# noce2/FluidFramework

Measured on AMD Instinct MI355X. Metric: sequenced merge-tree ops applied/sec (node) at 100k docs; bit-exact text+props, higher is better.
Workload: dtype int32; 1 GPU; c3: 100000 docs/GPU x 10000 sequenced ops, 8 writers, refSeq lag <= 64, insert 0.5 / remove 0.3 / annotate 0.2; docs_total=100000, docs_per_gpu=100000, ops_per_doc=10000, parallelism=doc-shard x1

## Files before the change

fluidframework_amd/__init__.py:

```python
import ctypes

import numpy as np

from . import _native
from .wire import CHECKSUM_DTYPE, OP_DTYPE, Batch, Interner

__all__ = ["MergeTreeBatch", "DeviceBatch", "Batch", "Interner", "DeltaLogOverflow"]


class DeltaLogOverflow(RuntimeError):

    def __init__(self, msg, records):
        super().__init__(msg)
        self.records = records


class PinnedArray:

    def __init__(self, lib, n, dtype):
        dt = np.dtype(dtype)
        nbytes = max(int(n), 1) * dt.itemsize
        self.lib = lib
        self.p = lib.mt_host_alloc(nbytes)
        if not self.p:
# ... 354 lines not shown
        off = np.zeros(self.n_docs + 1, dtype=np.int64)
        self._check(self.lib.mt_generated_seeds_docs(self.h, ctypes.byref(c), doc_base, _native.ptr(ids),
                                                     _native.ptr(off), None), "mt_generated_seeds")
        seed = np.zeros(max(int(off[-1]), 1), dtype=np.uint16)
        self._check(self.lib.mt_generated_seeds_docs(self.h, ctypes.byref(c), doc_base, _native.ptr(ids),
                                                     _native.ptr(off), _native.ptr(seed)), "mt_generated_seeds")
        return off, seed

    def sync(self):
        self._check(self.lib.mt_sync(self.h), "mt_sync")

    def last_hbm_docs(self):
        out = np.zeros(8, dtype=np.uint32)
        self._check(self.lib.mt_last_hbm_docs(self.h, _native.ptr(out)), "mt_last_hbm_docs")
        return dict(total=int(out[0]), spilled=int(out[1]), segments=int(out[2]), blocks=int(out[3]), heap=int(out[4]),
                    text=int(out[5]), props=int(out[6]), at_load=int(out[7]))

    def last_paged_peaks(self):
        out = np.zeros(5, dtype=np.uint32)
        self._check(self.lib.mt_last_paged_peaks(self.h, _native.ptr(out)), "mt_last_paged_peaks")
        return dict(pages=int(out[0]), unsettled=int(out[1]), heap=int(out[2]), segments=int(out[3]),
                    tight_handovers=int(out[4]))

    def last_grown(self):
        out = np.zeros(6, dtype=np.uint32)
        self._check(self.lib.mt_last_grown(self.h, _native.ptr(out)), "mt_last_grown")
        return dict(zip(["grown", "rounds", "in_big_region", "pages", "unsettled", "heap"], (int(x) for x in out)))

    def last_kernel_ms(self):
        return float(self.lib.mt_last_kernel_ms(self.h))

    def set_stream_priority(self, priority):
        self._check(self.lib.mt_set_stream_priority(self.h, int(priority)), "mt_set_stream_priority")

    def last_load_ms(self):
        return float(self.lib.mt_last_load_ms(self.h))

    def status(self):
        out = np.zeros(self.n_docs, dtype=np.int32)
        self._check(self.lib.mt_get_status(self.h, _native.ptr(out)), "mt_get_status")
        return out

    def get_length(self, doc):
        out = ctypes.c_uint32()
        self._check(self.lib.mt_get_length(self.h, doc, ctypes.byref(out)), "mt_get_length")
        return out.value
# ... 291 lines not shown
```

fluidframework_amd/_native.py:

```python
import ctypes
import os

import numpy as np

from .wire import CHECKSUM_DTYPE, OP_DTYPE

HERE = os.path.dirname(os.path.abspath(__file__))
MT_E_INVALID, MT_E_HIP, MT_E_NOMEM, MT_E_NODEVICE, MT_E_OVERFLOW, MT_E_STALE_VIEW = -1, -2, -3, -4, -5, -6
LIB_PATH = os.environ.get("MT_LIB_PATH") or os.path.join(HERE, "libmtreplay.so")


class MtOptions(ctypes.Structure):
    _fields_ = [("device", ctypes.c_int32), ("seg_capacity", ctypes.c_int32),
                ("block_capacity", ctypes.c_int32), ("heap_capacity", ctypes.c_int32),
                ("text_capacity", ctypes.c_int32), ("props_capacity", ctypes.c_int32),
                ("delta_log_capacity", ctypes.c_int32), ("lds_seg_capacity", ctypes.c_int32),
                ("page_capacity", ctypes.c_int32), ("page_heap_capacity", ctypes.c_int32),
                ("unsettled_capacity", ctypes.c_int32), ("uid_capacity", ctypes.c_int32),
                ("lds_page_capacity", ctypes.c_int32), ("lds_unsettled_capacity", ctypes.c_int32),
                ("lds_page_heap_capacity", ctypes.c_int32), ("lds_narrow_overlap", ctypes.c_int32),
                ("delta_log_mode", ctypes.c_int32), ("live_client", ctypes.c_int32),
                ("live_group_capacity", ctypes.c_int32), ("paged_slices", ctypes.c_int32),
                ("segment_ordinals", ctypes.c_int32), ("overlap_arena_capacity", ctypes.c_int32)]

# ... 28 lines not shown
    ("mt_num_docs", _U32, [_P]),
    ("mt_load_initial_text", _I, [_P, _P, _P]),
    ("mt_start_collaboration", _I, [_P, _P, _P]),
    ("mt_reset", _I, [_P]),
    ("mt_apply_ops", _I, [_P, _P, _P, _U64, _P, _U64, _P, _U64]),
    ("mt_load_snapshots", _I, [_P, _P, _P, _P, _U64, _P, _U64, _P, _U64, _P, _P]),
    ("mt_extract_snapshots", _I, [_P, _P, _P, _P, _P, _P, _P]),
    ("mt_snapshots_upload", _P, [_P, _P, _P, _P, _U64, _P, _U64, _P, _U64, _P, _P]),
    ("mt_snapshots_upload_range", _P, [_P, _U32, _U32, _P, _P, _P, _U64, _P, _U64, _P, _U64, _P, _P]),
    ("mt_snapshots_load_async", _I, [_P, _P]),
    ("mt_snapshots_free", None, [_P]),
    ("mt_batch_upload", _P, [_P, _P, _P, _U64, _P, _U64, _P, _U64]),
    ("mt_batch_apply_async", _I, [_P, _P]),
    ("mt_batch_num_ops", _U64, [_P]),
    ("mt_batch_free", None, [_P]),
    ("mt_host_alloc", ctypes.c_void_p, [ctypes.c_uint64]),
    ("mt_host_free", None, [ctypes.c_void_p]),
    ("mt_sync", _I, [_P]),
    ("mt_last_kernel_ms", ctypes.c_float, [_P]),
    ("mt_set_stream_priority", ctypes.c_int, [_P, ctypes.c_int]),
    ("mt_last_load_ms", ctypes.c_float, [_P]),
    ("mt_last_hbm_docs", _I, [_P, _P]),
    ("mt_last_paged_peaks", _I, [_P, _P]),
    ("mt_last_grown", _I, [_P, _P]),
    ("mt_generate", _P, [_P, _P, _U32, _P]),
    ("mt_generate_docs", _P, [_P, _P, _U32, _P, _P, _P]),
    ("mt_generated_seeds_docs", _I, [_P, _P, _U32, _P, _P, _P]),
    ("mt_generated_seeds", _I, [_P, _P, _U32, _P, _P]),
    ("mt_batch_sizes", _I, [_P, _P, _P, _P]),
    ("mt_batch_download", _I, [_P, _P, _P, _P, _P]),
    ("mt_get_status", _I, [_P, _P]),
    ("mt_get_length", _I, [_P, _U32, _P]),
    ("mt_get_text", _I, [_P, _U32, _P, _U32, _P]),
    ("mt_get_texts", _I, [_P, _U32, _P, _P, _P, ctypes.c_uint16, _P, _P, _U64]),
    ("mt_get_texts_device", _I, [_P, _U32, _P, _P, _P, ctypes.c_uint16, _P, _P, _U64]),
    ("mt_last_text_ms", _I, [_P, _P]),
    ("mt_get_prop_runs", _I, [_P, _U32, _P, _U32, _P, _P, _U32, _P]),
    ("mt_get_segments", _I, [_P, _U32, _P, _U32, _P, _P, _U32, _P]),
    ("mt_get_segment_props", _I, [_P, _U32, _U32, _P, _U32, _P]),
    ("mt_get_all_segment_props", _I, [_P, _U32, _P, ctypes.c_uint64, _P]),
    ("mt_get_overlap_arena", _I, [_P, _U32, _P]),
    ("mt_get_delta_log", _I, [_P, _U32, _P, _U32, _P]),
    ("mt_delta_log_reset", _I, [_P]),
    ("mt_debug_raw", _I, [_P, _U32, _P, _U32, _P, _P]),
    ("mt_debug_prof", _I, [_P, _P, _I]),
    ("mt_maintenance_counts", _I, [_P, _P]),
# ... 41 lines not shown
```

fluidframework_amd/csrc/mt_device.h:

```cpp
#pragma once
#include <hip/hip_runtime.h>
#include <stdint.h>

#include "../../include/mt_types.h"

#define MT_WAVE 64
#define MT_LV 8
#define MT_MAXN 8
#define MT_HALF 4
#define MT_GRAN 256
#define MT_ZAMBONI 2
#define MT_KMAX 8
#define MT_PREC (1 + 2 * MT_KMAX)
#define MT_RSEQ_NONE ((int32_t)0x80000000)
#define MT_MARKER_BIT 0x80000000u
#define MT_SCOUR_UNDEF ((int8_t)-1)
#define MT_DOC_RETRY 100

typedef unsigned long long u64;
typedef int v4i __attribute__((ext_vector_type(4)));
typedef unsigned v4u __attribute__((ext_vector_type(4)));
typedef int v2i __attribute__((ext_vector_type(2)));

struct DocHdr {
    int32_t n_seg, depth, heap_n, cur_seq;
    int32_t min_seq, text_top, text_half, props_top;
    int32_t props_half, next_uid, status, dlog_n;
    int32_t n_blk[MT_LV];
    u64 delta_hash;
    int32_t n_ops, pad0;
    int32_t pad[8];
};
static_assert(sizeof(DocHdr) == 128, "DocHdr size");
// ... 273 lines not shown
```

fluidframework_amd/csrc/mt_engine.h:

```cpp
#pragma once
#include <type_traits>

#include "mt_device.h"

#define LDS_AS __attribute__((address_space(3)))
#define GLB_AS __attribute__((address_space(1)))

template <bool kLogT> struct TierLdsT {
    static constexpr bool kLds = true;
    static constexpr bool kLog = kLogT;
    static constexpr bool kPaged = false;
    static constexpr bool kLive = false;
    static constexpr int kOvlBits = 32;
    static constexpr bool kMayGrow = false;
    static constexpr bool kOvf = false;
    typedef uint32_t O_v;
    typedef LDS_AS v4i *A_t;
    typedef LDS_AS uint32_t *O_t;
    typedef LDS_AS v4u *B_t;
    typedef LDS_AS v2i *H_t;
};
template <bool kLogT> struct TierGlbT {
    static constexpr bool kLds = false;
    static constexpr bool kLog = kLogT;
// ... 1562 lines not shown
            sa = d.A[s + k];
            so = d.O[s + k];
            sb = d.Bv[s + k];
            if constexpr (T::kLive) sp = pq_get(d, s + k);
            if (ordon(d)) soc = d.os[s + k];
        }
        const int dst = s + __popcll(m_keep & ((1ull << k) - 1ull));
        wsync<T>();
        if (surv) {
            d.A[dst] = sa;
            d.O[dst] = so;
            d.Bv[dst] = sb;
            if constexpr (T::kLive) pq_put(d, dst, sp);
            if (ordon(d)) d.os[dst] = soc;
        }
        wsync<T>();
        if (ordon(d)) gsync();
        seg_move_left(d, e, cntb - keep);
        d.n -= cntb - keep;
    }
    return keep;
}

TD int scour_range(DocT<T> &d, int s, int b0, int nbk) {
    int tot = 0;
    for (int q = 0; q < nbk; q++) tot += cntr(d, 0, b0 + q);
    const int k = lane();
    bool serial = tot > MT_WAVE;
    const bool in = k < tot;
    v4i a = d.A[in ? s + k : s];
    v4u b = d.Bv[in ? s + k : s];
    int start = 0;
    {
        int st = 0;
        for (int q = 0; q < nbk; q++) {
            if (k >= st) start = st;
            st += cntr(d, 0, b0 + q);
        }
    }
    const bool removed = a.z != MT_RSEQ_NONE;
    const bool marker = (b.z & MT_MARKER_BIT) != 0;
    bool pend = false;
    if constexpr (T::kLive) pend = in && pq_any(pq_get(d, in ? s + k : s));
    const bool cand = in && !pend && !removed && a.y <= d.min_seq;
    if (!serial) {
        const bool need_nl = cand && !marker && a.x > 0 && !(b.w & SEGF_NL_KNOWN);
        if (ballot(need_nl)) {
            P2_T0(9)
            gsync_rd();
            if (need_nl) {
                const uint16_t ch = text_base(d, d.text_half)[b.x + a.x - 1];
                b.w = (b.w & ~SEGF_NL) | SEGF_NL_KNOWN | (ch == '\n' ? SEGF_NL : 0u);
                d.Bv[s + k].w = b.w;
            }
            wsync<T>();
            P2_T1(9)
        }
    }
    const u64 m_cand = ballot(cand);
    const u64 m_mark = ballot(in && marker);
    const u64 m_nl = ballot(in && (b.w & SEGF_NL) != 0);
    const uint32_t pprops = (uint32_t)__shfl_up((int)b.y, 1, MT_WAVE);
    const bool pc = k > 0 && ((m_cand >> (k - 1)) & 1ull);
    const bool pm = k > 0 && ((m_mark >> (k - 1)) & 1ull);
    const bool pn = k > 0 && ((m_nl >> (k - 1)) & 1ull);
#ifdef MT_NO_Q4
    const u64 m_nm = 0;
#else
    const u64 m_nm = ballot(in && (b.w & SEGF_NOMATCH) != 0);
#endif
    const bool nm = ((m_nm >> k) & 1ull) || (k > 0 && ((m_nm >> (k - 1)) & 1ull));
    bool join = cand && pc && k != start && !marker && !pm && !pn && a.x > 0;
    if (join && (nm || pprops != b.y)) join = match_props(d, pprops, b.y, nm);
    const u64 m_join = ballot(join);
    if (!serial && ballot(join && a.x > MT_GRAN)) serial = true;
    if (serial) {
        int pos = s, kept_all = 0;
        for (int q = 0; q < nbk; q++) {
            const int old = cntr(d, 0, b0 + q);
            const int kept = scour_block(d, pos, pos + old);
            if (d.status) return kept_all;
            wsync<T>();
            if (lane() == 0) lvl(d, 0)[b0 + q] = (uint8_t)kept;
            wsync<T>();
            pos += kept;
            kept_all += kept;
        }
        return kept_all;
    }
    const bool unlink = in && !pend && removed && a.z <= d.min_seq;
    const bool surv = in && !unlink && !join;
    if (T::kLog) {
        d.m_unlink += __popcll(ballot(unlink));
        d.m_append += __popcll(m_join);
    }
    const u64 m_surv = ballot(surv);
    scour_events(d, a, b, ballot(unlink), m_join, m_surv, s, tot, start);
    const u64 above = (k < 63) ? (m_join >> (k + 1)) : 0ull;
    const u64 m_grp = ballot(surv && (above & 1ull));
    P2_T0(10)
    if (m_grp) {
        mark_dirty(d, s);
        const int L = wave_scan_incl(in ? a.x : 0);
        const int gend = k + __ffsll((long long)~above) - 1;
        const int Lend = __shfl(L, gend < MT_WAVE ? gend : MT_WAVE - 1, MT_WAVE);
        const int glen = Lend - L + (in ? a.x : 0);
        int totc = 0;
        for (u64 g = m_grp; g; g &= g - 1) {
            const int gl = bcast(glen, first_lane(g));
            totc += gl + text_slack(gl);
        }
        if (!text_ensure(d, totc)) return tot;
        gsync_rd();
        for (u64 g = m_grp; g; g &= g - 1) {
            const int kk = first_lane(g);
            const int gk = bcast(glen, kk);
            const int ge = bcast(gend, kk);
            const v4u bk = uni4(d.Bv[s + kk]);
            const int ak = uni(d.A[s + kk].x);
            const uint32_t kslack = bk.w >> SEGF_SLACK_SHIFT;
            const bool mem = k > kk && k <= ge;
            const v4u bm = d.Bv[mem ? s + k : s];
            const int Lm = L - (in ? a.x : 0);
            const int Lk = bcast(L, kk) - ak;
            const int rel = Lm - Lk;
            const bool contig_lane = !mem || (int)bm.x == (int)bk.x + rel;
            const bool contig = !ballot(!contig_lane);
            const int add = gk - ak;
            const uint32_t lastw = (uint32_t)bcast((int)bm.w, ge);
            const uint32_t nonl = (bk.w & SEGF_NONL) && !ballot(mem && !(bm.w & SEGF_NONL)) ? SEGF_NONL : 0u;
            uint32_t newoff = bk.x, newslack = lastw >> SEGF_SLACK_SHIFT;
            if (!contig) {
                int dst;
                bool move_keeper = false;
                if ((uint32_t)add <= kslack) {
                    dst = (int)bk.x + ak;
                    newslack = kslack - (uint32_t)add;
                } else if ((int)bk.x + ak == d.text_top) {
                    dst = d.text_top;
                    newslack = (uint32_t)text_slack(gk);
// ... 1053 lines not shown
```

fluidframework_amd/csrc/mt_kernels.h:

```cpp
#pragma once
#include "../../include/mt_replay.h"
#include "mt_paged.h"

__device__ static void init_doc_hdr(const DevState &st, int doc, int len) {
    DocHdr h;
    memset(&h, 0, sizeof(h));
    h.depth = 1;
    h.n_blk[0] = 1;
    h.text_top = len;
    h.props_top = 1;
    h.next_uid = 2;
    h.delta_hash = MT_FNV_OFF;
    h.status = len > st.T ? MT_DOC_CAPACITY : 0;
    const size_t S = st.S;
    if (len > 0) {
        h.n_seg = 1;
        st.segA[doc * S] = v4i{len, 0, MT_RSEQ_NONE, pack_cli(-1, 0)};
        st.segO[doc * S] = 0ull;
        st.segB[doc * S] = v4u{0u, 0u, 1u, 0u};
        if (st.segP) {
            u64 *w = (u64 *)(st.segP + doc * S);
            w[0] = w[1] = w[2] = w[3] = 0ull;
        }
    }
// ... 387 lines not shown
    gen_end(g, used_out, doc);
    if (T::kLds && d.status == MT_DOC_RETRY) {
        if (lane() == 0) st.retry[doc] = 1;
        return;
    }
    if (lane() == 0) {
        if (d.status) fail_out[doc] = d.status;
        if (!T::kLds) st.retry[doc] = 0;
    }
    store_doc(d, st, doc);
}

template <class T>
__device__ __forceinline__ void pg_peaks(const DevState &st, PagedDoc<T> &pd, int pk_ut, int pk_heap) {
    const int np = nbr(pd.up, 1);
    int ns = 0;
    for (int q = lane(); q < np; q += MT_WAVE) ns += pm_nseg(pd, pd.up.dir[q]);
    ns = wave_sum(ns);
    if (lane() == 0) {
        atomicMax(st.stats + 8, (uint32_t)np);
        atomicMax(st.stats + 9, (uint32_t)pk_ut);
        atomicMax(st.stats + 10, (uint32_t)pk_heap);
        atomicMax(st.stats + 11, (uint32_t)ns);
    }
}
#ifndef MT_PAGED_WAVES
#define MT_PAGED_WAVES 3
#endif
#ifndef MT_HM_WAVES
#define MT_HM_WAVES 2
#endif
#ifndef MT_FULL_WAVES
#define MT_FULL_WAVES 2
#endif
#ifndef MT_PACKED_WAVES
#define MT_PACKED_WAVES 2
#endif
template <class T> constexpr int paged_waves() {
    return T::kHM ? MT_HM_WAVES
                  : (T::kMayGrow ? MT_FULL_WAVES : (T::kPacked ? MT_PACKED_WAVES : MT_PAGED_WAVES));
}
#if MT_PAGED_WAVES > 0
#define MT_PAGED_WPE __attribute__((amdgpu_waves_per_eu(paged_waves<T>())))
#else
#define MT_PAGED_WPE
#endif
// ... 249 lines not shown
```

fluidframework_amd/csrc/mt_paged.h:

```cpp
#pragma once
#include "mt_engine.h"

#ifdef MT_PROF
#define PG_T0(k) const unsigned long long _pt##k = __builtin_amdgcn_s_memtime();
#define PG_T1(k)                                                         \
    if (lane() == 0) {                                                   \
        pd.w.prof[k] += __builtin_amdgcn_s_memtime() - _pt##k;           \
        pd.w.prof[64 + k] += 1ull;                                       \
    }
#define PG_CNT(k)                                                        \
    if (lane() == 0) pd.w.prof[64 + k] += 1ull;
#else
#define PG_T0(k)
#define PG_T1(k)
#define PG_CNT(k)
#endif

template <class T> struct PagedDoc {
    DocT<T> w;
    DocT<T> up;
    LDS_AS PageMeta *meta;
    GLB_AS PageMeta *gmeta;
    LDS_AS int *pvl;
    LDS_AS int *cob;
// ... 43 lines not shown
    int grow;
    int packed;
};

#define PW_B 16
#define MT_PK_MASKS 256

struct PagedLayout {
    uint32_t offWA, offWB, offWO, offWcnt, offWflg, offWends, offWscr, offWnb;
    uint32_t offUcnt, offUnb, offDir, offMeta, offCob, offHeap, offUpage, offUA, offUO, offGen, offProf,
        total;
};
static __host__ __device__ inline PagedLayout paged_layout(int PP, int PH, int UT, int gen_words, int ob,
                                                           bool packed = false, bool hm = false) {
    PagedLayout L;
    uint32_t o = 0;
    L.offWA = o; o += 16u * MT_PG_SLOTS;
    L.offWB = o; o += 16u * MT_PG_SLOTS;
    L.offWO = o; o += (uint32_t)ob * MT_PG_SLOTS;
    L.offUA = o; o += (packed ? 12u : 16u) * UT;
    o = (o + 7u) & ~7u;
    L.offUO = o; o += packed ? 8u * MT_PK_MASKS + MT_PK_MASKS / 8 : ((((uint32_t)ob * UT) + 7u) & ~7u);
    L.offHeap = o; o += 8u * (PH + 1);
    L.offMeta = o; o += hm ? 0u : (uint32_t)sizeof(PageMeta) * PP;
    L.offUpage = o; o += packed ? 0u : (2u * UT + 3u) & ~3u;
    L.offCob = o; o += hm ? 8u * (uint32_t)((PP + 63) / 64) + 4u * 64 : 4u * PP;
    L.offWscr = o; o += 64u * 4;
    L.offWnb = o; o += MT_LV * 4;
    L.offUnb = o; o += MT_LV * 4;
    L.offGen = o; o += 4u * gen_words;
    L.offDir = o; o += 2u * PP;
    L.offWends = o; o += 2u * PW_B;
    L.offWcnt = o; o += (uint32_t)MT_LV * PW_B;
    L.offWflg = o; o += PW_B;
    L.offUcnt = o; o += (uint32_t)(pcnt_bytes(PP) - PP);
#ifdef MT_PROF
    o = (o + 7u) & ~7u;
    L.offProf = o; o += 128u * 8;
#else
    L.offProf = 0;
#endif
    L.total = (o + 15u) & ~15u;
    return L;
}

TD PagedDoc<T> &pdoc(DocT<T> &w) { return *reinterpret_cast<PagedDoc<T> *>(&w); }
template <class T> __device__ __forceinline__ PagedCaps eff_caps(PagedCaps pc) {
// ... 1125 lines not shown
    for (int j = 0; j < nch; j++) {
        const int pg = uni(up.dir[c0 + j]);
        if (lane() == 0) pm_set_ns(pd, pg, 0, 0);
        wsync<T>();
    }
    blk_replace(up, 1, c0, nch, k, base, extra);
    if (up.status) {
        pg_fail_cap(w, 7);
        return;
    }
    for (int m = 0; m < k; m++)
        if (lane() == 0) up.dir[c0 + m] = (uint16_t)newp[m];
    if (lane() == 0) lvl(up, 2)[P] = (uint8_t)k;
    wsync<T>();
    pg_cob_rebuild(pd);
    int top_l = 2, top_b = P;
    if (k < MT_HALF && 3 < up.depth) pack_counts(up, 2, P, top_l, top_b);
    if (up.status) {
        if (w.status == 0) w.cap_cause = up.cap_cause;
        fail(w, MT_DOC_INTERNAL);
        return;
    }
    if (ordon(w)) ord_canon(up, top_l, top_b);
}

TD void pg_zamboni_impl(PagedDoc<T> &pd);
TD void pg_zamboni(PagedDoc<T> &pd) {
    PG_T0(12)
    pg_zamboni_impl(pd);
    PG_T1(12)
}
TD void pg_zamboni_impl(PagedDoc<T> &pd) {
    DocT<T> &w = pd.w;
    pd.vvalid = 0;
    for (int it = 0; it < MT_ZAMBONI && w.status == 0; it++) {
        if (w.heap_n == 0) break;
        const v2i top = heap_top(w);
        if (top.x > w.min_seq) break;
        const uint32_t uid = (uint32_t)top.y;
        if (uid >= (uint32_t)pd.UM) {
            FAIL_INTERNAL(w);
            return;
        }
#ifdef MT_ZPF
        const int gpg = uid == (uint32_t)pd.zuid ? pd.zpv : (int)pd.gumap[uid];
        pd.zuid = 0;
// ... 18 lines not shown
                    PG_CNT(19)
                    continue;
                }
                v4i a = v4i{0, 0, 0, 0};
                u64 o = 0;
                v4u b = v4u{0, 0, 0, 0};
                uint32_t bc = 0, f2 = 0;
                int ob = 0;
                pg_win_fetch(pd, pg, a, o, b);
                pg_win_fetch_blocks(pd, pg, bc, f2, ob);
                if ((((uint32_t)bcast((int)f2, 0)) >> 24) == 0) {
                    PG_CNT(19)
                    continue;
                }
                PG_CNT(18)
                pg_win_flush(pd);
                if (w.status) return;
                pg_win_place(pd, pg, a, o, b, bc, f2, ob);
            } else {
                if (pg == pd.cur || pg >= pd.PP || uni(pm_nseg(pd, pg)) == 0) {
                    PG_CNT(19)
                    continue;
                }
                PG_CNT(18)
                pg_win_switch(pd, pg);
                if (w.status) return;
            }
            i = find_uid(w, uid);
            if (i < 0) {
                PG_CNT(19)
                continue;
            }
        }
        PG_T1(4)
        int bstart;
        const int b = blk_find(w, 0, i, true, bstart);
        if (b < 0) {
            FAIL_INTERNAL(w);
            return;
        }
        const int f = flgr(w, b);
        const int old = cntr(w, 0, b);
        if (f == 0) {
            PG_CNT(20)
            continue;
        }
// ... 175 lines not shown
        const int ns = uni(pm_nseg(pd, pg));
        if (i < ns) {
            GLB_AS v4u *b = pd.gB + (size_t)pg * MT_PG_SLOTS + i;
            const uint32_t nid = (uint32_t)(uni((int)first[pg]) + i);
            v4u bv = *b;
            bv.z = nid | (bv.z & MT_MARKER_BIT);
            *b = bv;
            if (nid < (uint32_t)pd.UM) pd.gumap[nid] = (uint16_t)pg;
        }
    }
    w.next_uid = carry;
    if (w.next_uid + 8 > pd.UM && !soft) pg_fail_cap(w, 9);
    gsync();
    wsync<T>();
}

TD bool pg_room(PagedDoc<T> &pd, const mt_op_rec &op) {
    const bool range = op.kind == MT_OP_REMOVE || op.kind == MT_OP_ANNOTATE;
    const int span = range ? min(max(op.pos2 - op.pos1, 0), 1 << 20) : 0;
    const int ut_b = op.kind == MT_OP_INSERT ? 3 : (range ? 2 + span : (op.kind == MT_OP_LOAD_REMOVED ? 1 : 0));
    const int hp_b = op.kind == MT_OP_INSERT ? 1 : (range ? 1 + span : 0);
    if (T::kOvlBits < 64 && op.kind == MT_OP_REMOVE && oslot_short(pd.w, op_cli(op))) return false;
    if (T::kPacked && op.seq - pd.sbase > 65000) return false;
    if (pd.ut_n + pd.wgrow + ut_b > pd.UT) return false;
    if constexpr (T::kPacked) {
        const int need = pd.wgrow + ut_b;
        if (tab_mfree(pd) < need) {
            tab_mgc(pd);
            if (tab_mfree(pd) < need) return false;
        }
    }
    if (pd.w.heap_n + hp_b > pd.PH) return false;
    if (nbr(pd.up, 1) + 8 > pd.PP) return false;
    for (int l = 2; l < pd.up.depth; l++)
        if (nbr(pd.up, l) + 4 > bcap(pd.up, l)) return false;
    pd.opbound = ut_b;
    pd.wgrow += ut_b;
    return true;
}
TD void pg_apply_op_impl(PagedDoc<T> &pd, const OpIn &in, const GLB_AS uint16_t *tin, const GLB_AS uint32_t *pin);
TD void pg_apply_op(PagedDoc<T> &pd, const OpIn &in, const GLB_AS uint16_t *tin, const GLB_AS uint32_t *pin) {
    PG_T0(15)
    pg_apply_op_impl(pd, in, tin, pin);
    PG_T1(15)
}
TD void pg_load_removed(PagedDoc<T> &pd, const mt_op_rec &op) {
    DocT<T> &w = pd.w;
// ... 549 lines not shown
    pd.upage = (LDS_AS uint16_t *)(smem + L.offUpage);
    pd.uA = (LDS_AS v4i *)(smem + L.offUA);
    pd.uO = (LDS_AS typename T::O_v *)(smem + L.offUO);
    if constexpr (T::kPacked) {
        pd.uL = (LDS_AS uint32_t *)(smem + L.offUA);
        pd.uS = pd.uL + pc.UT;
        pd.uP = pd.uS + pc.UT;
        pd.sbase = h.cur_seq - 32000;
        pd.uM = (LDS_AS u64 *)(smem + L.offUO);
        pd.mbm = (LDS_AS uint32_t *)(smem + L.offUO + 8u * MT_PK_MASKS);
        if (lane() < MT_PK_MASKS / 32) pd.mbm[lane()] = lane() == 0 ? 1u : 0u;
        if (lane() == 0) pd.uM[0] = 0;
    }
    pd.cur = -1;
    pd.cur_pos = -1;
    pd.dirty = 0;
    pd.tdirty = 0;
    pd.vvalid = 0;
    pd.wgrow = 0;
    pd.opbound = 0;
    pd.zuid = 0;
    pd.zpv = 0;
    pd.press = 0;
    pd.ovf_top = MT_OVF_HDR;
    pd.ovf_last = 0;
    pd.ovf_maxn = 0;
    pd.ovf_half = 0;
    pd.ovf_made = 0;
    pd.ovf_peak = 0;
    if constexpr (T::kOvf) {
        if (pd.govf) {
            const GLB_AS uint32_t *hw = (const GLB_AS uint32_t *)pd.govf;
            pd.ovf_top = max((int)hw[0], MT_OVF_HDR);
            pd.ovf_last = (int)hw[1];
            pd.ovf_maxn = (int)hw[2];
            pd.ovf_made = hw[4];
            pd.ovf_peak = (int)hw[5];
            pd.ovf_half = ((int)hw[3] & 1) && pd.ovf_top > mt_ovf_mid(pd.OA) ? 1 : 0;
        }
    }
}

TD void pg_mark_free(PagedDoc<T> &pd) {
    const int np = nbr(pd.up, 1);
    pd.vvalid = 0;
    for (int base = 0; base < pd.PP; base += MT_WAVE)
// ... 300 lines not shown
```

fluidframework_amd/csrc/mt_replay.hip:

```cpp
#include <hip/hip_runtime.h>

#include <algorithm>
#include <cstdlib>
#include <cstdio>
#include <cstring>
#include <string>
#include <vector>

#include "../../include/mt_replay.h"
#include "mt_kernels.h"
#include "mt_variants.h"
#ifdef MT_SINGLE_TU
#define MT_VARIANT_DEF(n, k) const void *mtk_##n() { return (const void *)k; }
MT_VARIANTS(MT_VARIANT_DEF)
#endif

__global__ void __launch_bounds__(MT_WAVE) k_init(DevState st, const int64_t *seed_off,
                                                  const uint16_t *seed) {
    const int doc = blockIdx.x;
    if (doc >= st.n_docs) return;
    oslot_reset(st, doc);
    if (st.bslot && lane() == 0) st.bslot[doc] = -1;
    const int64_t s0 = seed_off ? seed_off[doc] : 0, s1 = seed_off ? seed_off[doc + 1] : 0;
    const int len = (int)(s1 - s0);
// ... 942 lines not shown
            h->pg_resident = per_cu * cus;
        }
    }
    const size_t N = n_docs;
    bool ok = true;
    auto alloc = [&](void **p, size_t bytes) {
        if (!ok) return;
        if (hipMalloc(p, bytes ? bytes : 16) != hipSuccess) ok = false;
    };
    alloc((void **)&st.hdr, N * sizeof(DocHdr));
    alloc((void **)&st.segA, N * st.S * sizeof(int4));
    alloc((void **)&st.segO, N * st.S * sizeof(u64));
    alloc((void **)&st.segB, N * st.S * sizeof(uint4));
    alloc((void **)&st.cnt, N * MT_LV * st.B);
    alloc((void **)&st.flg, N * st.B);
    alloc((void **)&st.heap, N * (size_t)(st.H + 1) * sizeof(int2));
    alloc((void **)&st.oslot, N * (size_t)(2 * MT_OSLOTS) * sizeof(int32_t));
    alloc((void **)&st.text, N * 2 * (size_t)st.T * sizeof(uint16_t));
    alloc((void **)&st.props, N * 2 * (size_t)st.P * MT_PREC * sizeof(uint32_t));
    if (st.DL) alloc((void **)&st.dlog, N * (size_t)st.DL * sizeof(int32_t));
    alloc((void **)&h->d_sums, N * sizeof(mt_checksum));
    alloc((void **)&st.retry, N * sizeof(int32_t));
    alloc((void **)&st.resume, N * sizeof(int64_t));
    alloc((void **)&st.stats, 16 * sizeof(uint32_t));
#ifdef MT_PROF
    alloc((void **)&st.prof, 128 * sizeof(unsigned long long));
    if (ok) ok = hipMemset(st.prof, 0, 128 * sizeof(unsigned long long)) == hipSuccess;
#endif
    if (h->ordinals) {
        alloc((void **)&st.ordS, N * (size_t)st.S * sizeof(uint16_t));
        alloc((void **)&st.ordB, N * (size_t)MT_LV * st.B * sizeof(uint16_t));
    }
    if (h->live) {
        alloc((void **)&st.live, N * 4 * sizeof(int32_t));
        st.LG = std::min(std::max(o.live_group_capacity > 0 ? o.live_group_capacity : 1024, 16), 65535);
        alloc((void **)&st.grp, N * (size_t)(st.LG + 1) * MT_GRP_WORDS * sizeof(int32_t));
        alloc((void **)&st.segP, N * (size_t)st.S * sizeof(PendQ));
    }
    if (st.PP > 0) {
        const size_t slots = N * (size_t)st.PP * MT_PG_SLOTS;
        alloc((void **)&st.pgA, slots * sizeof(int4));
        alloc((void **)&st.pgO, slots * sizeof(u64));
        alloc((void **)&st.pgB, slots * sizeof(uint4));
        alloc((void **)&st.pgMeta, N * st.PP * sizeof(PageMeta));
        alloc((void **)&st.pgDir, N * st.PP * sizeof(uint16_t));
        alloc((void **)&st.pgCnt, N * MT_LV * (size_t)st.PP);
        alloc((void **)&st.pgHeap, N * (size_t)(st.PH + 1) * sizeof(int2));
// ... 233 lines not shown
        launch_replay_paged(MTK(P_LOG), g, blk, lb, h->stream, h->st, b->ops, b->off, b->text,
                           b->props, res, pc, sl);
    else if (pc.narrow)
        launch_replay_paged(MTK(P_NARROW), g, blk, lb, h->stream, h->st, b->ops, b->off,
                           b->text, b->props, res, pc, sl);
    else if (hm)
        launch_replay_paged(MTK(P_HM), g, blk, lb, h->stream, h->st, b->ops, b->off, b->text,
                           b->props, res, pc, sl);
    else
        launch_replay_paged(MTK(P_FULL), g, blk, lb, h->stream, h->st, b->ops, b->off, b->text,
                           b->props, res, pc, sl);
    HIPCHK(h, hipGetLastError());
    return 0;
}

int mt_batch_apply_async(mt_handle *h, const mt_batch *b) {
    if (!h || !b || b->n_docs != h->n_docs) return MT_E_INVALID;
    if (h->pending) {
        const int rc = mt_settle(h);
        if (rc) return rc;
    }
    h->st.order = b->order;
    HIPCHK(h, hipSetDevice(h->device));
    HIPCHK(h, hipMemsetAsync(h->st.stats, 0, 16 * sizeof(uint32_t), h->stream));
    HIPCHK(h, hipEventRecord(h->ev0, h->stream));
    if (h->lds.S > 0) {
        if (h->live && h->st.DL)
            launch_replay(MTK(R_LIVELDS_LOG), dim3(h->n_docs), dim3(MT_WAVE),
                               tier_lds_bytes(true, h->lds, 0), h->stream, h->st, b->ops, b->off, b->text, b->props,
                               h->lds);
        else if (h->live)
            launch_replay(MTK(R_LIVELDS), dim3(h->n_docs), dim3(MT_WAVE),
                               tier_lds_bytes(true, h->lds, 0), h->stream, h->st, b->ops, b->off, b->text, b->props,
                               h->lds);
        else if (h->st.DL)
            launch_replay(MTK(R_LDS_LOG), dim3(h->n_docs), dim3(MT_WAVE), tier_lds_bytes(true, h->lds, 0),
                               h->stream, h->st, b->ops, b->off, b->text, b->props, h->lds);
        else if (h->wpg == 2)
            launch_replay(MTK(R_LDS2), dim3((h->n_docs + 1) / 2), dim3(2 * MT_WAVE),
                               2 * tier_lds_bytes(true, h->lds, 0), h->stream, h->st, b->ops, b->off, b->text, b->props,
                               h->lds);
        else
            launch_replay(MTK(R_LDS), dim3(h->n_docs), dim3(MT_WAVE), tier_lds_bytes(true, h->lds, 0),
                               h->stream, h->st, b->ops, b->off, b->text, b->props, h->lds);
        HIPCHK(h, hipGetLastError());
    } else {
        HIPCHK(h, hipMemsetD32Async((hipDeviceptr_t)h->st.retry, 1, h->n_docs, h->stream));
// ... 564 lines not shown
    HIPCHK(h, hipMemcpy(out, h->st.stats, 8 * sizeof(uint32_t), hipMemcpyDeviceToHost));
    return 0;
}

int mt_last_grown(mt_handle *h, uint32_t *out) {
    if (!h || !out) return MT_E_INVALID;
    SETTLE(h);
    uint32_t in_big = 0;
    for (int32_t x : h->bslot_h) in_big += x >= 0;
    out[0] = h->grown_last;
    out[1] = h->grow_rounds_last;
    out[2] = in_big;
    out[3] = (uint32_t)h->big_caps.PP;
    out[4] = (uint32_t)h->big_caps.UT;
    out[5] = (uint32_t)h->big_caps.PH;
    return 0;
}

int mt_last_paged_peaks(mt_handle *h, uint32_t *out) {
    if (!h || !out) return MT_E_INVALID;
    HIPCHK(h, hipSetDevice(h->device));
    SETTLE(h);
    HIPCHK(h, hipMemcpy(out, h->st.stats + 8, 5 * sizeof(uint32_t), hipMemcpyDeviceToHost));
    return 0;
}

int mt_apply_ops(mt_handle *h, const int64_t *doc_op_off, const mt_op_rec *ops, uint64_t n_ops,
                 const uint16_t *text, uint64_t text_len, const uint32_t *props,
                 uint64_t props_len) {
    if (!h) return MT_E_INVALID;
    h->err.clear();
    mt_batch *b = mt_batch_upload(h, doc_op_off, ops, n_ops, text, text_len, props, props_len);
    if (!b) return h->err.rfind("mt_batch_upload: device", 0) == 0 ? MT_E_NOMEM : MT_E_INVALID;
    int rc = mt_batch_apply_async(h, b);
    if (rc == 0) rc = mt_sync(h);
    mt_batch_free(b);
    return rc;
}

struct mt_snapshots {
    int device = 0;
    uint32_t doc_lo = 0, n_docs = 0;
    int64_t *off = nullptr;
    int32_t *nh = nullptr, *min_seq = nullptr, *cur_seq = nullptr;
    mt_seg_rec *segs = nullptr;
    uint16_t *text = nullptr;
// ... 341 lines not shown
    b->n_ops = off[N];
    b->text_len = off[N] * cfg->text_max + N;
    b->props_len = off[N] * (1 + 2 * (int64_t)cfg->max_keys_per_op) + N;
    int32_t *d_fail = nullptr, *d_trace = nullptr;
    int64_t *d_used = nullptr;
    if (view_len_trace && hipMalloc(&d_trace, std::max<int64_t>(b->n_ops, 1) * 16) != hipSuccess) {
        delete b;
        return nullptr;
    }
    bool ok = hipMalloc(&b->off, (N + 1) * sizeof(int64_t)) == hipSuccess &&
              hipMalloc(&b->ops, std::max<int64_t>(b->n_ops, 1) * sizeof(mt_op_rec)) == hipSuccess &&
              hipMalloc(&b->text, b->text_len * 2) == hipSuccess &&
              hipMalloc(&b->props, b->props_len * 4) == hipSuccess &&
              hipMalloc(&d_fail, N * 4) == hipSuccess && hipMalloc(&d_used, N * 16) == hipSuccess;
    if (ok) {
        ok = hipMemcpy(b->off, off.data(), (N + 1) * 8, hipMemcpyHostToDevice) == hipSuccess &&
             hipMemset(d_fail, 0, N * 4) == hipSuccess && set_order(b, off.data());
        h->st.gen_off = ops_per_doc ? b->off : nullptr;
    }
    int32_t *d_ids = nullptr;
    if (ok && doc_ids)
        ok = hipMalloc(&d_ids, N * 4) == hipSuccess && hipMemcpy(d_ids, doc_ids, N * 4, hipMemcpyHostToDevice) == hipSuccess;
    h->st.gen_ids = d_ids;
    if (ok) ok = hipMemsetAsync(h->st.stats, 0, 16 * sizeof(uint32_t), h->stream) == hipSuccess;
    if (ok) {
        const int gw = 2 * (cfg->writers + 1);
        if (h->lds.S > 0) {
            launch_generate(MTK(G_LDS), dim3(h->n_docs), dim3(MT_WAVE), tier_lds_bytes(true, h->lds, gw),
                               h->stream, h->st, *cfg, doc_index_base, b->ops, b->text, b->props, tstride,
                               pstride, d_fail, d_trace, d_used, h->lds);
            ok = hipGetLastError() == hipSuccess;
        } else {
            ok = hipMemsetD32Async((hipDeviceptr_t)h->st.retry, 1, h->n_docs, h->stream) == hipSuccess;
        }
        if (ok && h->st.PP > 0) {
            const PagedCaps *tiers[2] = {h->pg_tight.PP ? &h->pg_tight : nullptr, &h->pg_full};
            for (const PagedCaps *pc : tiers) {
                if (!pc || !ok) continue;
                const size_t lb = paged_layout(pc->PP, pc->PH, pc->UT, gw, pc->narrow ? 4 : 8).total;
                if (pc->narrow)
                    launch_generate_paged(MTK(GP_NARROW), dim3(h->n_docs), dim3(MT_WAVE), lb,
                                       h->stream, h->st, *cfg, doc_index_base, b->ops, b->text, b->props, tstride,
                                       pstride, d_fail, d_trace, d_used, *pc);
                else
                    launch_generate_paged(MTK(GP_FULL), dim3(h->n_docs), dim3(MT_WAVE), lb,
                                       h->stream, h->st, *cfg, doc_index_base, b->ops, b->text, b->props, tstride,
                                       pstride, d_fail, d_trace, d_used, *pc);
// ... 976 lines not shown
```

include/mt_replay.h:

```cpp
#ifndef MT_REPLAY_H
#define MT_REPLAY_H
#include <stddef.h>
#include <stdint.h>

#include "mt_types.h"

#ifdef __cplusplus
extern "C" {
#endif

#define MT_E_INVALID (-1)
#define MT_E_HIP (-2)
#define MT_E_NOMEM (-3)
#define MT_E_NODEVICE (-4)
#define MT_E_OVERFLOW (-5)
#define MT_E_STALE_VIEW (-6)

typedef struct mt_handle mt_handle;
typedef struct mt_batch mt_batch;

typedef struct mt_options {
    int32_t device;
    int32_t seg_capacity;
    int32_t block_capacity;
// ... 50 lines not shown
                                        const int32_t *n_header, const mt_seg_rec *segs, uint64_t n_segs,
                                        const uint16_t *text, uint64_t text_len, const uint32_t *props,
                                        uint64_t props_len, const int32_t *min_seq, const int32_t *cur_seq);
int mt_snapshots_load_async(mt_handle *h, const mt_snapshots *s);
void mt_snapshots_free(mt_snapshots *s);
float mt_last_load_ms(mt_handle *h);

int mt_extract_snapshots(mt_handle *h, int64_t *io, mt_seg_rec *recs, uint16_t *text, uint32_t *props,
                         int32_t *min_seq, int32_t *cur_seq);

mt_batch *mt_batch_upload(mt_handle *h, const int64_t *doc_op_off, const mt_op_rec *ops,
                          uint64_t n_ops, const uint16_t *text, uint64_t text_len,
                          const uint32_t *props, uint64_t props_len);
int mt_batch_apply_async(mt_handle *h, const mt_batch *b);
uint64_t mt_batch_num_ops(const mt_batch *b);
void mt_batch_free(mt_batch *b);
void *mt_host_alloc(uint64_t bytes);
void mt_host_free(void *p);
int mt_sync(mt_handle *h);
float mt_last_kernel_ms(const mt_handle *h);
int mt_set_stream_priority(mt_handle *h, int priority);
int mt_last_hbm_docs(mt_handle *h, uint32_t *out);
int mt_last_paged_peaks(mt_handle *h, uint32_t *out);

int mt_last_grown(mt_handle *h, uint32_t *out);

mt_batch *mt_generate(mt_handle *h, const mt_gen_cfg *cfg, uint32_t doc_index_base,
                      int32_t *view_len_trace );
mt_batch *mt_generate_docs(mt_handle *h, const mt_gen_cfg *cfg, uint32_t doc_index_base,
                           const int32_t *ops_per_doc, const int32_t *doc_ids, int32_t *view_len_trace);
int mt_generated_seeds_docs(mt_handle *h, const mt_gen_cfg *cfg, uint32_t doc_index_base, const int32_t *doc_ids,
                            int64_t *seed_off, uint16_t *seed_text);
int mt_generated_seeds(mt_handle *h, const mt_gen_cfg *cfg, uint32_t doc_index_base,
                       int64_t *seed_off, uint16_t *seed_text);
int mt_batch_sizes(const mt_batch *b, uint64_t *n_ops, uint64_t *text_len, uint64_t *props_len);
int mt_batch_download(const mt_batch *b, int64_t *doc_op_off, mt_op_rec *ops, uint16_t *text,
                      uint32_t *props);

int mt_get_status(mt_handle *h, int32_t *out_status);
int mt_get_length(mt_handle *h, uint32_t doc, uint32_t *out);
int mt_get_text(mt_handle *h, uint32_t doc, uint16_t *out, uint32_t cap, uint32_t *out_len);
int mt_get_texts(mt_handle *h, uint32_t n, const uint32_t *docs, const int32_t *start,
                 const int32_t *end, uint16_t marker_unit, int64_t *off, uint16_t *out, uint64_t cap);
int mt_get_texts_device(mt_handle *h, uint32_t n, const uint32_t *docs, const int32_t *start,
                        const int32_t *end, uint16_t marker_unit, void *off_dev, void *out_dev, uint64_t cap);
int mt_last_text_ms(mt_handle *h, float *out );
// ... 60 lines not shown
```

Before: 159.8 million ops/s.

## Scour paged blocks in place during zamboni instead of switching page windows

Splits scour_range into reusable plan/group/merge helpers and adds an in-place zamboni path for paged documents. When the target block can be compacted without structural change, it is rewritten directly in its global page instead of paying for a full window switch. When the unsettled table fills, the window is flushed early rather than failing the op. A small stats counter pair and an API for them are added. The risk is extra divergence and fallback cost when the in-place conditions fail, plus subtle correctness risk in the compaction.

After: 162.3 million ops/s (median of 6 runs). 1.02x the previous value.

```diff
diff --git a/fluidframework_amd/__init__.py b/fluidframework_amd/__init__.py
--- a/fluidframework_amd/__init__.py
+++ b/fluidframework_amd/__init__.py
@@ -400,6 +400,11 @@
         return dict(pages=int(out[0]), unsettled=int(out[1]), heap=int(out[2]), segments=int(out[3]),
                     tight_handovers=int(out[4]))
 
+    def last_zamboni(self):
+        out = np.zeros(2, dtype=np.uint32)
+        self._check(self.lib.mt_last_zamboni(self.h, _native.ptr(out)), "mt_last_zamboni")
+        return {"in_place": int(out[0]), "fallback": int(out[1])}
+
     def last_grown(self):
         out = np.zeros(6, dtype=np.uint32)
         self._check(self.lib.mt_last_grown(self.h, _native.ptr(out)), "mt_last_grown")
diff --git a/fluidframework_amd/_native.py b/fluidframework_amd/_native.py
--- a/fluidframework_amd/_native.py
+++ b/fluidframework_amd/_native.py
@@ -74,6 +74,7 @@
     ("mt_last_load_ms", ctypes.c_float, [_P]),
     ("mt_last_hbm_docs", _I, [_P, _P]),
     ("mt_last_paged_peaks", _I, [_P, _P]),
+    ("mt_last_zamboni", _I, [_P, _P]),
     ("mt_last_grown", _I, [_P, _P]),
     ("mt_generate", _P, [_P, _P, _U32, _P]),
     ("mt_generate_docs", _P, [_P, _P, _U32, _P, _P, _P]),
diff --git a/fluidframework_amd/csrc/mt_device.h b/fluidframework_amd/csrc/mt_device.h
--- a/fluidframework_amd/csrc/mt_device.h
+++ b/fluidframework_amd/csrc/mt_device.h
@@ -9,6 +9,7 @@
 #define MT_MAXN 8
 #define MT_HALF 4
 #define MT_GRAN 256
+#define MT_STATS_WORDS 20
 #define MT_ZAMBONI 2
 #define MT_KMAX 8
 #define MT_PREC (1 + 2 * MT_KMAX)
diff --git a/fluidframework_amd/csrc/mt_engine.h b/fluidframework_amd/csrc/mt_engine.h
--- a/fluidframework_amd/csrc/mt_engine.h
+++ b/fluidframework_amd/csrc/mt_engine.h
@@ -1608,40 +1608,24 @@
     return keep;
 }
 
-TD int scour_range(DocT<T> &d, int s, int b0, int nbk) {
-    int tot = 0;
-    for (int q = 0; q < nbk; q++) tot += cntr(d, 0, b0 + q);
+struct ScourPlan {
+    u64 m_join, m_unlink, m_surv;
+    bool big;
+};
+TD ScourPlan scour_plan(DocT<T> &d, const v4i &a, v4u &b, bool in, bool pend, int start, bool &nl_res) {
     const int k = lane();
-    bool serial = tot > MT_WAVE;
-    const bool in = k < tot;
-    v4i a = d.A[in ? s + k : s];
-    v4u b = d.Bv[in ? s + k : s];
-    int start = 0;
-    {
-        int st = 0;
-        for (int q = 0; q < nbk; q++) {
-            if (k >= st) start = st;
-            st += cntr(d, 0, b0 + q);
-        }
-    }
     const bool removed = a.z != MT_RSEQ_NONE;
     const bool marker = (b.z & MT_MARKER_BIT) != 0;
-    bool pend = false;
-    if constexpr (T::kLive) pend = in && pq_any(pq_get(d, in ? s + k : s));
     const bool cand = in && !pend && !removed && a.y <= d.min_seq;
-    if (!serial) {
-        const bool need_nl = cand && !marker && a.x > 0 && !(b.w & SEGF_NL_KNOWN);
-        if (ballot(need_nl)) {
-            P2_T0(9)
-            gsync_rd();
-            if (need_nl) {
-                const uint16_t ch = text_base(d, d.text_half)[b.x + a.x - 1];
-                b.w = (b.w & ~SEGF_NL) | SEGF_NL_KNOWN | (ch == '\n' ? SEGF_NL : 0u);
-                d.Bv[s + k].w = b.w;
-            }
-            wsync<T>();
-            P2_T1(9)
-        }
+    nl_res = cand && !marker && a.x > 0 && !(b.w & SEGF_NL_KNOWN);
+    if (ballot(nl_res)) {
+        P2_T0(9)
+        gsync_rd();
+        if (nl_res) {
+            const uint16_t ch = text_base(d, d.text_half)[b.x + a.x - 1];
+            b.w = (b.w & ~SEGF_NL) | SEGF_NL_KNOWN | (ch == '\n' ? SEGF_NL : 0u);
+        }
+        P2_T1(9)
     }
     const u64 m_cand = ballot(cand);
     const u64 m_mark = ballot(in && marker);
@@ -1658,8 +1642,130 @@
     const bool nm = ((m_nm >> k) & 1ull) || (k > 0 && ((m_nm >> (k - 1)) & 1ull));
     bool join = cand && pc && k != start && !marker && !pm && !pn && a.x > 0;
     if (join && (nm || pprops != b.y)) join = match_props(d, pprops, b.y, nm);
-    const u64 m_join = ballot(join);
-    if (!serial && ballot(join && a.x > MT_GRAN)) serial = true;
+    ScourPlan p;
+    p.m_join = ballot(join);
+    p.big = ballot(join && a.x > MT_GRAN) != 0;
+    const bool unlink = in && !pend && removed && a.z <= d.min_seq;
+    p.m_unlink = ballot(unlink);
+    p.m_surv = ballot(in && !unlink && !join);
+    return p;
+}
+struct ScourGroups {
+    u64 m_grp;
+    int L, gend, glen, totc;
+};
+__device__ __forceinline__ ScourGroups scour_groups(const v4i &a, bool in, u64 m_join, u64 m_surv) {
+    const int k = lane();
+    const u64 above = (k < 63) ? (m_join >> (k + 1)) : 0ull;
+    ScourGroups g;
+    g.m_grp = ballot(((m_surv >> k) & 1ull) && (above & 1ull));
+    g.L = g.gend = g.glen = g.totc = 0;
+    if (g.m_grp) {
+        g.L = wave_scan_incl(in ? a.x : 0);
+        g.gend = k + __ffsll((long long)~above) - 1;
+        const int Lend = __shfl(g.L, g.gend < MT_WAVE ? g.gend : MT_WAVE - 1, MT_WAVE);
+        g.glen = Lend - g.L + (in ? a.x : 0);
+        for (u64 q = g.m_grp; q; q &= q - 1) {
+            const int gl = bcast(g.glen, first_lane(q));
+            g.totc += gl + text_slack(gl);
+        }
+    }
+    return g;
+}
+TD void scour_merge(DocT<T> &d, v4i &a, v4u &b, bool in, const ScourGroups &g) {
+    const int k = lane();
+    const v4i a0 = a;
+    const v4u bm = b;
+    const int L = g.L;
+    for (u64 q = g.m_grp; q; q &= q - 1) {
+        const int kk = first_lane(q);
+        const int gk = bcast(g.glen, kk);
+        const int ge = bcast(g.gend, kk);
+        const v4u bk = v4u{(uint32_t)bcast((int)bm.x, kk), (uint32_t)bcast((int)bm.y, kk),
+                           (uint32_t)bcast((int)bm.z, kk), (uint32_t)bcast((int)bm.w, kk)};
+        const int ak = bcast(a0.x, kk);
+        const uint32_t kslack = bk.w >> SEGF_SLACK_SHIFT;
+        const bool mem = k > kk && k <= ge;
+        const int Lm = L - (in ? a0.x : 0);
+        const int Lk = bcast(L, kk) - ak;
+        const int rel = Lm - Lk;
+        const bool contig_lane = !mem || (int)bm.x == (int)bk.x + rel;
+        const bool contig = !ballot(!contig_lane);
+        const int add = gk - ak;
+        const uint32_t lastw = (uint32_t)bcast((int)bm.w, ge);
+        const uint32_t nonl = (bk.w & SEGF_NONL) && !ballot(mem && !(bm.w & SEGF_NONL)) ? SEGF_NONL : 0u;
+        uint32_t newoff = bk.x, newslack = lastw >> SEGF_SLACK_SHIFT;
+        if (!contig) {
+            int dst;
+            bool move_keeper = false;
+            if ((uint32_t)add <= kslack) {
+                dst = (int)bk.x + ak;
+                newslack = kslack - (uint32_t)add;
+            } else if ((int)bk.x + ak == d.text_top) {
+                dst = d.text_top;
+                newslack = (uint32_t)text_slack(gk);
+                d.text_top += add + (int)newslack;
+            } else {
+                newoff = (uint32_t)d.text_top;
+                dst = d.text_top + ak;
+                move_keeper = true;
+                newslack = (uint32_t)text_slack(gk);
+                d.text_top += gk + (int)newslack;
+            }
+            GLB_AS uint16_t *tb = text_base(d, d.text_half);
+            const int t0 = move_keeper ? 0 : ak;
+            for (int base = t0; base < gk; base += MT_WAVE) {
+                const int t = base + lane();
+                int src = 0;
+                if (t < ak) {
+                    src = (int)bk.x + t;
+                } else {
+                    for (int j = kk + 1; j <= ge; j++) {
+                        const int rj = bcast(Lm, j) - Lk;
+                        if (t >= rj) src = bcast((int)bm.x, j) + (t - rj);
+                    }
+                }
+                uint16_t ch = 0;
+                if (t < gk) ch = tb[src];
+                if (t < gk) tb[(move_keeper ? (int)newoff : dst - ak) + t] = ch;
+            }
+        }
+        if (k == kk) {
+            a.x = gk;
+            b.x = newoff;
+            b.w = (lastw & (SEGF_NL_KNOWN | SEGF_NL)) | nonl | (newslack << SEGF_SLACK_SHIFT);
+        }
+    }
+}
+
+TD int scour_range(DocT<T> &d, int s, int b0, int nbk) {
+    int tot = 0;
+    for (int q = 0; q < nbk; q++) tot += cntr(d, 0, b0 + q);
+    const int k = lane();
+    bool serial = tot > MT_WAVE;
+    const bool in = k < tot;
+    v4i a = d.A[in ? s + k : s];
+    v4u b = d.Bv[in ? s + k : s];
+    int start = 0;
+    {
+        int st = 0;
+        for (int q = 0; q < nbk; q++) {
+            if (k >= st) start = st;
+            st += cntr(d, 0, b0 + q);
+        }
+    }
+    bool pend = false;
+    if constexpr (T::kLive) pend = in && pq_any(pq_get(d, in ? s + k : s));
+    ScourPlan pl = ScourPlan{0ull, 0ull, 0ull, false};
+    if (!serial) {
+        bool nl_res;
+        pl = scour_plan(d, a, b, in, pend, start, nl_res);
+        if (ballot(nl_res)) {
+            if (nl_res) d.Bv[s + k].w = b.w;
+            wsync<T>();
+        }
+        serial = pl.big;
+    }
     if (serial) {
         int pos = s, kept_all = 0;
         for (int q = 0; q < nbk; q++) {
@@ -1674,34 +1780,24 @@
         }
         return kept_all;
     }
-    const bool unlink = in && !pend && removed && a.z <= d.min_seq;
-    const bool surv = in && !unlink && !join;
+    const u64 m_join = pl.m_join, m_surv = pl.m_surv;
+    const bool surv = (m_surv >> k) & 1ull;
     if (T::kLog) {
-        d.m_unlink += __popcll(ballot(unlink));
+        d.m_unlink += __popcll(pl.m_unlink);
         d.m_append += __popcll(m_join);
     }
-    const u64 m_surv = ballot(surv);
-    scour_events(d, a, b, ballot(unlink), m_join, m_surv, s, tot, start);
-    const u64 above = (k < 63) ? (m_join >> (k + 1)) : 0ull;
-    const u64 m_grp = ballot(surv && (above & 1ull));
+    scour_events(d, a, b, pl.m_unlink, m_join, m_surv, s, tot, start);
+    const ScourGroups g = scour_groups(a, in, m_join, m_surv);
     P2_T0(10)
-    if (m_grp) {
+    if (g.m_grp) {
         mark_dirty(d, s);
-        const int L = wave_scan_incl(in ? a.x : 0);
-        const int gend = k + __ffsll((long long)~above) - 1;
-        const int Lend = __shfl(L, gend < MT_WAVE ? gend : MT_WAVE - 1, MT_WAVE);
-        const int glen = Lend - L + (in ? a.x : 0);
-        int totc = 0;
-        for (u64 g = m_grp; g; g &= g - 1) {
-            const int gl = bcast(glen, first_lane(g));
-            totc += gl + text_slack(gl);
-        }
-        if (!text_ensure(d, totc)) return tot;
+        if (!text_ensure(d, g.totc)) return tot;
         gsync_rd();
-        for (u64 g = m_grp; g; g &= g - 1) {
-            const int kk = first_lane(g);
-            const int gk = bcast(glen, kk);
-            const int ge = bcast(gend, kk);
+        const int L = g.L;
+        for (u64 q = g.m_grp; q; q &= q - 1) {
+            const int kk = first_lane(q);
+            const int gk = bcast(g.glen, kk);
+            const int ge = bcast(g.gend, kk);
             const v4u bk = uni4(d.Bv[s + kk]);
             const int ak = uni(d.A[s + kk].x);
             const uint32_t kslack = bk.w >> SEGF_SLACK_SHIFT;
diff --git a/fluidframework_amd/csrc/mt_kernels.h b/fluidframework_amd/csrc/mt_kernels.h
--- a/fluidframework_amd/csrc/mt_kernels.h
+++ b/fluidframework_amd/csrc/mt_kernels.h
@@ -433,6 +433,11 @@
         atomicMax(st.stats + 9, (uint32_t)pk_ut);
         atomicMax(st.stats + 10, (uint32_t)pk_heap);
         atomicMax(st.stats + 11, (uint32_t)ns);
+        if constexpr (pg_zinplace<T>()) {
+            const uint32_t zi = pg_zcount(pd)[0], zf = pg_zcount(pd)[1];
+            if (zi) atomicAdd(st.stats + 16, zi);
+            if (zf) atomicAdd(st.stats + 17, zf);
+        }
     }
 }
 #ifndef MT_PAGED_WAVES
diff --git a/fluidframework_amd/csrc/mt_paged.h b/fluidframework_amd/csrc/mt_paged.h
--- a/fluidframework_amd/csrc/mt_paged.h
+++ b/fluidframework_amd/csrc/mt_paged.h
@@ -89,7 +89,7 @@
     o = (o + 7u) & ~7u;
     L.offUO = o; o += packed ? 8u * MT_PK_MASKS + MT_PK_MASKS / 8 : ((((uint32_t)ob * UT) + 7u) & ~7u);
     L.offHeap = o; o += 8u * (PH + 1);
-    L.offMeta = o; o += hm ? 0u : (uint32_t)sizeof(PageMeta) * PP;
+    L.offMeta = o; o += hm ? 0u : (uint32_t)sizeof(PageMeta) * PP + 8u;
     L.offUpage = o; o += packed ? 0u : (2u * UT + 3u) & ~3u;
     L.offCob = o; o += hm ? 8u * (uint32_t)((PP + 63) / 64) + 4u * 64 : 4u * PP;
     L.offWscr = o; o += 64u * 4;
@@ -1261,6 +1261,93 @@
         return;
     }
     if (ordon(w)) ord_canon(up, top_l, top_b);
+}
+
+TD LDS_AS uint32_t *pg_zcount(PagedDoc<T> &pd) { return (LDS_AS uint32_t *)(pd.meta + pd.PP); }
+template <class T> constexpr bool pg_zinplace() {
+#ifdef MT_NO_ZINPLACE
+    return false;
+#else
+    return !T::kLog && !T::kHM && !T::kLive;
+#endif
+}
+TD bool pg_scour_inplace(PagedDoc<T> &pd, int pg, uint32_t uid) {
+    DocT<T> &w = pd.w;
+    const int k = lane();
+    const int n = uni(pm_nseg(pd, pg)), nb = uni(pm_nblk(pd, pg));
+    v4i a = v4i{0, 0, 0, 0};
+    v4u b = v4u{0, 0, 0, 0};
+    if (k < n) {
+        a = pd.gA[(size_t)pg * MT_PG_SLOTS + k];
+        b = pd.gB[(size_t)pg * MT_PG_SLOTS + k];
+    }
+    uint32_t bc, f2;
+    pm_blocks(pd, pg, bc, f2);
+    bc = (uint32_t)uni((int)bc);
+    f2 = (uint32_t)uni((int)f2);
+    const u64 hit = ballot(k < n && (b.z & ~MT_MARKER_BIT) == uid);
+    if (!hit) {
+        PG_CNT(19)
+        return false;
+    }
+    const int i = first_lane(hit);
+    int q = 0, bstart = 0;
+    while (q < nb && q < 8 && i >= bstart + pm_bc_of(bc, q)) {
+        bstart += pm_bc_of(bc, q);
+        q++;
+    }
+    if (q >= nb || q >= 8) {
+        FAIL_INTERNAL(w);
+        return false;
+    }
+    if (pm_fl_of(f2, q) == 0) {
+        PG_CNT(20)
+        return false;
+    }
+    const int cnt = pm_bc_of(bc, q);
+    if (pd.up.depth < 2 || bstart + cnt > n) return true;
+    const bool in = k >= bstart && k < bstart + cnt;
+    bool nl_res;
+    const ScourPlan pl = scour_plan(w, a, b, in, false, bstart, nl_res);
+    const int keep = __popcll(pl.m_surv);
+    if (pl.big || (keep < cnt && keep < MT_HALF)) return true;
+    const ScourGroups g = scour_groups(a, in, pl.m_join, pl.m_surv);
+    if (g.m_grp && w.text_top + g.totc > w.T_cap) return true;
+    PG_CNT(21)
+    PG_CNT(37)
+    if (k == 0) pg_zcount(pd)[0]++;
+    const uint32_t nbc = (bc & ~(15u << (4 * q))) | ((uint32_t)keep << (4 * q));
+    const uint32_t nf2 = (f2 & ~(3u << (2 * q))) | (1u << (2 * q));
+    if (g.m_grp) {
+        gsync_rd();
+        scour_merge(w, a, b, in, g);
+    }
+    if (keep < cnt || g.m_grp) {
+        const u64 blk = ((1ull << cnt) - 1ull) << bstart;
+        const u64 chg = g.m_grp | (blk & ~pl.m_surv);
+        const int first = __ffsll((long long)chg) - 1;
+        const bool surv = (pl.m_surv >> k) & 1ull;
+        const int dst = in ? bstart + __popcll(pl.m_surv & ((1ull << k) - 1ull)) : k - (cnt - keep);
+        const bool st = k < n && k >= first && (in ? surv : keep < cnt);
+        const bool mv = st && dst != k;
+        u64 o = 0;
+        if (mv) o = pd.gO[(size_t)pg * MT_PG_SLOTS + k];
+        asm volatile("" : "+v"(o));
+        if (st) {
+            pd.gA[(size_t)pg * MT_PG_SLOTS + dst] = a;
+            pd.gB[(size_t)pg * MT_PG_SLOTS + dst] = b;
+        }
+        if (mv) pd.gO[(size_t)pg * MT_PG_SLOTS + dst] = o;
+    } else {
+        PG_CNT(38)
+    }
+    if (k == 0) {
+        pd.meta[pg].bc = nbc;
+        pd.meta[pg].flg2 = (uint16_t)nf2;
+        pm_set_ns(pd, pg, n - (cnt - keep), nb);
+    }
+    wsync<T>();
+    return false;
 }
 
 TD void pg_zamboni_impl(PagedDoc<T> &pd);
@@ -1325,6 +1412,11 @@
                     PG_CNT(19)
                     continue;
                 }
+                if constexpr (pg_zinplace<T>()) {
+                    if (!pg_scour_inplace(pd, pg, uid)) continue;
+                    if (w.status) return;
+                    if (lane() == 0) pg_zcount(pd)[1]++;
+                }
                 PG_CNT(18)
                 pg_win_switch(pd, pg);
                 if (w.status) return;
@@ -1546,7 +1638,12 @@
     const int hp_b = op.kind == MT_OP_INSERT ? 1 : (range ? 1 + span : 0);
     if (T::kOvlBits < 64 && op.kind == MT_OP_REMOVE && oslot_short(pd.w, op_cli(op))) return false;
     if (T::kPacked && op.seq - pd.sbase > 65000) return false;
-    if (pd.ut_n + pd.wgrow + ut_b > pd.UT) return false;
+    if (pd.ut_n + pd.wgrow + ut_b > pd.UT) {
+        if (!pg_zinplace<T>() || pd.cur < 0 || !pd.dirty) return false;
+        pd.opbound = 0;
+        pg_win_flush(pd);
+        if (pd.w.status || pd.ut_n + pd.wgrow + ut_b > pd.UT) return false;
+    }
     if constexpr (T::kPacked) {
         const int need = pd.wgrow + ut_b;
         if (tab_mfree(pd) < need) {
@@ -2142,6 +2239,9 @@
     pd.zuid = 0;
     pd.zpv = 0;
     pd.press = 0;
+    if constexpr (!T::kHM) {
+        if (lane() == 0) pg_zcount(pd)[0] = pg_zcount(pd)[1] = 0;
+    }
     pd.ovf_top = MT_OVF_HDR;
     pd.ovf_last = 0;
     pd.ovf_maxn = 0;
diff --git a/fluidframework_amd/csrc/mt_replay.hip b/fluidframework_amd/csrc/mt_replay.hip
--- a/fluidframework_amd/csrc/mt_replay.hip
+++ b/fluidframework_amd/csrc/mt_replay.hip
@@ -988,7 +988,7 @@
     alloc((void **)&h->d_sums, N * sizeof(mt_checksum));
     alloc((void **)&st.retry, N * sizeof(int32_t));
     alloc((void **)&st.resume, N * sizeof(int64_t));
-    alloc((void **)&st.stats, 16 * sizeof(uint32_t));
+    alloc((void **)&st.stats, MT_STATS_WORDS * sizeof(uint32_t));
 #ifdef MT_PROF
     alloc((void **)&st.prof, 128 * sizeof(unsigned long long));
     if (ok) ok = hipMemset(st.prof, 0, 128 * sizeof(unsigned long long)) == hipSuccess;
@@ -1268,7 +1268,7 @@
     }
     h->st.order = b->order;
     HIPCHK(h, hipSetDevice(h->device));
-    HIPCHK(h, hipMemsetAsync(h->st.stats, 0, 16 * sizeof(uint32_t), h->stream));
+    HIPCHK(h, hipMemsetAsync(h->st.stats, 0, MT_STATS_WORDS * sizeof(uint32_t), h->stream));
     HIPCHK(h, hipEventRecord(h->ev0, h->stream));
     if (h->lds.S > 0) {
         if (h->live && h->st.DL)
@@ -1879,6 +1879,14 @@
     HIPCHK(h, hipSetDevice(h->device));
     SETTLE(h);
     HIPCHK(h, hipMemcpy(out, h->st.stats + 8, 5 * sizeof(uint32_t), hipMemcpyDeviceToHost));
+    return 0;
+}
+
+int mt_last_zamboni(mt_handle *h, uint32_t *out) {
+    if (!h || !out) return MT_E_INVALID;
+    HIPCHK(h, hipSetDevice(h->device));
+    SETTLE(h);
+    HIPCHK(h, hipMemcpy(out, h->st.stats + 16, 2 * sizeof(uint32_t), hipMemcpyDeviceToHost));
     return 0;
 }
 
@@ -2266,7 +2274,7 @@
     if (ok && doc_ids)
         ok = hipMalloc(&d_ids, N * 4) == hipSuccess && hipMemcpy(d_ids, doc_ids, N * 4, hipMemcpyHostToDevice) == hipSuccess;
     h->st.gen_ids = d_ids;
-    if (ok) ok = hipMemsetAsync(h->st.stats, 0, 16 * sizeof(uint32_t), h->stream) == hipSuccess;
+    if (ok) ok = hipMemsetAsync(h->st.stats, 0, MT_STATS_WORDS * sizeof(uint32_t), h->stream) == hipSuccess;
     if (ok) {
         const int gw = 2 * (cfg->writers + 1);
         if (h->lds.S > 0) {
diff --git a/include/mt_replay.h b/include/mt_replay.h
--- a/include/mt_replay.h
+++ b/include/mt_replay.h
@@ -96,6 +96,7 @@
 int mt_set_stream_priority(mt_handle *h, int priority);
 int mt_last_hbm_docs(mt_handle *h, uint32_t *out);
 int mt_last_paged_peaks(mt_handle *h, uint32_t *out);
+int mt_last_zamboni(mt_handle *h, uint32_t *out);
 
 int mt_last_grown(mt_handle *h, uint32_t *out);
 
```
